# src-d/kmcuda

Hardware: AMD Instinct MI355X
Metric: point-assignments/sec per Lloyd iter (8Mx256@1024) (higher is better)
Workload: dtype f32

## Files before the change

kmcuda_amd/csrc/update.hip:

```cpp
#include <stdio.h>
#include <stdlib.h>
#include <string.h>

#include <algorithm>

#include <rocprim/device/device_radix_sort.hpp>

#include "exact.hpp"
#include "kernels.hpp"

namespace kmx {

static unsigned bits_for(uint64_t maxval) {
  unsigned b = 1;
  while (b < 32 && (1ull << b) <= maxval) b++;
  return b;
}

size_t sort_temp_bytes(size_t n, uint32_t max_key) {
  size_t bytes = 0;
  (void)rocprim::radix_sort_pairs(nullptr, bytes, (const uint32_t *)nullptr, (uint32_t *)nullptr,
                                  (const uint32_t *)nullptr, (uint32_t *)nullptr, n, 0u, bits_for(max_key),
                                  (hipStream_t)0);
  return bytes;
}

__global__ void offsets_kernel(const uint32_t *__restrict__ keys_sorted, uint32_t n, uint32_t nkeys,
                               uint32_t *__restrict__ offsets) {
  const uint32_t k = blockIdx.x * blockDim.x + threadIdx.x;
  if (k > nkeys) return;
  uint32_t lo = 0, hi = n;
  while (lo < hi) {
    const uint32_t mid = lo + (hi - lo) / 2;
    if (keys_sorted[mid] < k) lo = mid + 1; else hi = mid;
  }
  offsets[k] = lo;
}

__global__ void cluster_keys_kernel(const uint32_t *__restrict__ assignments, uint32_t N, uint32_t K,
                                    uint32_t *__restrict__ keys, uint32_t *__restrict__ vals) {
  const uint32_t s = blockIdx.x * blockDim.x + threadIdx.x;
  if (s >= N) return;
  const uint32_t a = assignments[s];
  keys[s] = a < K ? a : K;
  vals[s] = s;
}

hipError_t launch_inverse_assignments(const uint32_t *assignments, uint32_t N, uint32_t K, uint32_t *keys_tmp,
                                      uint32_t *vals_tmp, uint32_t *keys_sorted, uint32_t *inv,
                                      uint32_t *offsets, void *temp, size_t temp_bytes, hipStream_t st) {
  hipLaunchKernelGGL(cluster_keys_kernel, dim3((N + 255) / 256), dim3(256), 0, st, assignments, N, K, keys_tmp,
                     vals_tmp);
  hipError_t e = rocprim::radix_sort_pairs(temp, temp_bytes, (const uint32_t *)keys_tmp, keys_sorted,
                                           (const uint32_t *)vals_tmp, inv, (size_t)N, 0u, bits_for(K), st);
  if (e != hipSuccess) return e;
  hipLaunchKernelGGL(offsets_kernel, dim3((K + 1 + 255) / 256), dim3(256), 0, st, keys_sorted, N, K, offsets);
  return hipGetLastError();
}

__global__ void knn_query_keys_kernel(const float *__restrict__ lb, size_t stride, const uint32_t *__restrict__ offsets,
                                      uint32_t K, uint32_t p_base, uint32_t p_end, uint32_t *__restrict__ keys,
                                      uint32_t *__restrict__ vals, int mode, const float *__restrict__ mydist,
                                      const float *__restrict__ R) {
  const uint32_t i = blockIdx.x * blockDim.x + threadIdx.x;
  if (i >= p_end - p_base) return;
  const uint32_t p = p_base + i;
  uint32_t lo = 0, hi = K;
  while (hi - lo > 1) {
    const uint32_t mid = (lo + hi) / 2;
    if (offsets[mid] <= p) lo = mid; else hi = mid;
  }
  const uint32_t cls = lo;
  vals[i] = p;
  if (mode == 2) {
    const float md = mydist[p];
    const uint32_t q = (md == md && md > 0.f) ? ((__float_as_uint(md) >> 16) & 0x7FFFu) : 0u;
    keys[i] = (cls << 15) | q;
    return;
  }
  float best = INFINITY;
  uint32_t arg = 0;
  for (uint32_t c = 0; c < K; c++) {
    const float v = lb[(size_t)c * stride + i];
    if (c != cls && v < best) { best = v; arg = c; }
  }
  if (mode == 3) {
    const float r = R[cls], md = mydist[p];
    uint32_t q = 0;
    if (r > 0.f && md == md) q = (uint32_t)fminf(63.f, fmaxf(0.f, md / r * 63.f));
    keys[i] = ((cls * K + arg) << 6) | q;
    return;
  }
  keys[i] = cls * K + arg;
}

bool launch_knn_query_order(const float *lb, size_t stride, const uint32_t *offsets, uint32_t K, uint32_t p_base,
                            uint32_t p_end, uint32_t *keys_tmp, uint32_t *vals_tmp, uint32_t *keys_sorted,
                            uint32_t *qperm, void *temp, size_t temp_bytes, hipStream_t st, int mode,
                            const float *mydist, const float *R) {
  if (p_end <= p_base || K > 65535u) return false;
  const uint64_t key_max = mode == 2 ? ((uint64_t)K << 15) : (mode == 3 ? ((uint64_t)K * K) << 6 : (uint64_t)K * K);
  if (key_max > 0xFFFFFFFFull) return false;
  const uint32_t n = p_end - p_base;
  size_t need = 0;
  if (rocprim::radix_sort_pairs(nullptr, need, (const uint32_t *)nullptr, (uint32_t *)nullptr, (const uint32_t *)nullptr,
                                (uint32_t *)nullptr, (size_t)n, 0u, bits_for(key_max), st) != hipSuccess ||
      need > temp_bytes)
    return false;
  hipLaunchKernelGGL(knn_query_keys_kernel, dim3((n + 255) / 256), dim3(256), 0, st, lb, stride, offsets, K, p_base,
                     p_end, keys_tmp, vals_tmp, mode, mydist, R);
  size_t bytes = temp_bytes;
  return rocprim::radix_sort_pairs(temp, bytes, (const uint32_t *)keys_tmp, keys_sorted, (const uint32_t *)vals_tmp,
                                   qperm, (size_t)n, 0u, bits_for(key_max), st) == hipSuccess &&
         hipGetLastError() == hipSuccess;
}

__global__ void knn_probe_keys_kernel(const uint32_t *__restrict__ probes, uint32_t pw, const uint32_t *__restrict__ qinv,
                                      const uint32_t *__restrict__ offsets, uint32_t K, uint32_t p_base, uint32_t p_end,
                                      uint32_t *__restrict__ keys, uint32_t *__restrict__ vals) {
  const uint32_t i = blockIdx.x * blockDim.x + threadIdx.x;
  if (i >= p_end - p_base) return;
  const uint32_t p = p_base + i;
  uint32_t lo = 0, hi = K;
  while (hi - lo > 1) {
    const uint32_t mid = (lo + hi) / 2;
    if (offsets[mid] <= p) lo = mid; else hi = mid;
  }
  const uint32_t second = probes[(size_t)qinv[p] * pw + 1];
  vals[i] = p;
  keys[i] = lo * (K + 1) + (second < K ? second : K);
}

bool launch_knn_probe_order(const uint32_t *probes, uint32_t pw, const uint32_t *qinv, const uint32_t *offsets,
                            uint32_t K, uint32_t p_base, uint32_t p_end, uint32_t *keys_tmp, uint32_t *vals_tmp,
                            uint32_t *keys_sorted, uint32_t *qperm, void *temp, size_t temp_bytes, hipStream_t st) {
  if (p_end <= p_base || pw < 2 || K > 65535u) return false;
  const uint64_t key_max = (uint64_t)K * (K + 1);
  if (key_max > 0xFFFFFFFFull) return false;
  const uint32_t n = p_end - p_base;
  size_t need = 0;
  if (rocprim::radix_sort_pairs(nullptr, need, (const uint32_t *)nullptr, (uint32_t *)nullptr, (const uint32_t *)nullptr,
                                (uint32_t *)nullptr, (size_t)n, 0u, bits_for(key_max), st) != hipSuccess ||
      need > temp_bytes)
    return false;
  hipLaunchKernelGGL(knn_probe_keys_kernel, dim3((n + 255) / 256), dim3(256), 0, st, probes, pw, qinv, offsets, K, p_base,
                     p_end, keys_tmp, vals_tmp);
  size_t bytes = temp_bytes;
  return rocprim::radix_sort_pairs(temp, bytes, (const uint32_t *)keys_tmp, keys_sorted, (const uint32_t *)vals_tmp,
                                   qperm, (size_t)n, 0u, bits_for(key_max), st) == hipSuccess &&
         hipGetLastError() == hipSuccess;
}

__global__ void move_events_kernel(const uint32_t *__restrict__ prev, const uint32_t *__restrict__ cur, uint32_t N,
                                   uint32_t K, uint32_t *__restrict__ keys, uint32_t *__restrict__ vals) {
  const uint32_t s = blockIdx.x * blockDim.x + threadIdx.x;
  if (s >= N) return;
  const uint32_t p = prev[s], a = cur[s];
  const bool moved = p != a;
  const uint32_t sentinel = 2u * K;
  keys[2 * (size_t)s] = (moved && a < K) ? 2u * a : sentinel;
  keys[2 * (size_t)s + 1] = (moved && p < K) ? 2u * p + 1u : sentinel;
  vals[2 * (size_t)s] = s;
  vals[2 * (size_t)s + 1] = s;
}

constexpr uint32_t kMoveRows = 1024;

__device__ __forceinline__ void move_flags(const uint32_t *__restrict__ prev, const uint32_t *__restrict__ cur,
                                           uint32_t s, uint32_t N, uint32_t K, uint32_t &p, uint32_t &a, bool &ein,
                                           bool &eout) {
  p = a = 0;
  ein = eout = false;
  if (s < N) {
    p = prev[s];
    a = cur[s];
    const bool moved = p != a;
    ein = moved && a < K;
    eout = moved && p < K;
  }
}

__global__ __launch_bounds__(256) void move_count_kernel(const uint32_t *__restrict__ prev,
                                                         const uint32_t *__restrict__ cur, uint32_t N, uint32_t K,
                                                         uint32_t *__restrict__ blockcnt) {
  uint32_t cnt = 0;
#pragma unroll
  for (uint32_t i = 0; i < kMoveRows / 256; i++) {
    uint32_t p, a;
    bool ein, eout;
    move_flags(prev, cur, blockIdx.x * kMoveRows + i * 256 + threadIdx.x, N, K, p, a, ein, eout);
    cnt += (uint32_t)ein + (uint32_t)eout;
  }
#pragma unroll
  for (int o = 32; o > 0; o >>= 1) cnt += __shfl_xor(cnt, o);
  __shared__ uint32_t w[4];
  if ((threadIdx.x & 63) == 0) w[threadIdx.x >> 6] = cnt;
  __syncthreads();
  if (threadIdx.x == 0) blockcnt[blockIdx.x] = w[0] + w[1] + w[2] + w[3];
}

__global__ __launch_bounds__(1024) void move_scan_kernel(uint32_t *__restrict__ blockcnt, uint32_t nb,
                                                         uint32_t *__restrict__ total) {
  __shared__ uint32_t wsum[16];
  __shared__ uint32_t carry_s;
  const uint32_t lane = threadIdx.x & 63, wave = threadIdx.x >> 6;
  if (threadIdx.x == 0) carry_s = 0;
  __syncthreads();
  for (uint32_t base = 0; base < nb; base += 1024) {
    const uint32_t i = base + threadIdx.x;
    const uint32_t v = i < nb ? blockcnt[i] : 0u;
    uint32_t inc = v;
#pragma unroll
    for (int o = 1; o < 64; o <<= 1) {
      const uint32_t t = __shfl_up(inc, o);
      if ((int)lane >= o) inc += t;
    }
    if (lane == 63) wsum[wave] = inc;
    __syncthreads();
    uint32_t wbase = 0, all = 0;
#pragma unroll
    for (uint32_t k = 0; k < 16; k++) {
      const uint32_t t = wsum[k];
      if (k < wave) wbase += t;
      all += t;
    }
    const uint32_t carry = carry_s;
    if (i < nb) blockcnt[i] = carry + wbase + inc - v;
    __syncthreads();
    if (threadIdx.x == 0) carry_s = carry + all;
    __syncthreads();
  }
  if (threadIdx.x == 0) total[0] = carry_s;
}

__global__ __launch_bounds__(256) void move_write_kernel(const uint32_t *__restrict__ prev,
                                                         const uint32_t *__restrict__ cur, uint32_t N, uint32_t K,
                                                         const uint32_t *__restrict__ blockoff,
                                                         uint32_t *__restrict__ keys, uint32_t *__restrict__ vals) {
  __shared__ uint32_t wcnt[4];
  const uint32_t lane = threadIdx.x & 63, wave = threadIdx.x >> 6;
  uint32_t off = blockoff[blockIdx.x];
#pragma unroll
  for (uint32_t i = 0; i < kMoveRows / 256; i++) {
    const uint32_t s = blockIdx.x * kMoveRows + i * 256 + threadIdx.x;
    uint32_t p, a;
    bool ein, eout;
    move_flags(prev, cur, s, N, K, p, a, ein, eout);
    const unsigned long long min = __ballot(ein), mout = __ballot(eout);
    const unsigned long long lower = (1ull << lane) - 1ull;
    const uint32_t rank = (uint32_t)__popcll(min & lower) + (uint32_t)__popcll(mout & lower);
    if (lane == 0) wcnt[wave] = (uint32_t)__popcll(min) + (uint32_t)__popcll(mout);
    __syncthreads();
    uint32_t wbase = 0, all = 0;
#pragma unroll
    for (uint32_t k = 0; k < 4; k++) {
      if (k < wave) wbase += wcnt[k];
      all += wcnt[k];
    }
    const size_t at = (size_t)off + wbase + rank;
    if (ein) { keys[at] = 2u * a; vals[at] = s; }
    if (eout) { keys[at + (ein ? 1 : 0)] = 2u * p + 1u; vals[at + (ein ? 1 : 0)] = s; }
    off += all;
    __syncthreads();
  }
}

constexpr uint32_t kSumThreads = 1024;
constexpr uint32_t kBucketCapMax = 4096;

uint32_t move_bucket_cap(uint32_t N, uint32_t K) {
  uint32_t cap = 32;
  while (cap < kBucketCapMax && (uint64_t)cap * 2 * K <= (uint64_t)N) cap <<= 1;
  return cap;
}

struct SumArgs {
  const float *samples;
  uint32_t N, D, K;
  const uint32_t *prev, *cur;
  uint32_t *cursors;
  uint32_t stride;
  const uint32_t *bucket_rows;
  uint32_t cap;
  uint32_t *overflow;
  const uint32_t *rows_sorted, *offsets2;
  double *delta;
  int32_t *dcount;
  double *tail;
  const uint32_t *counters;
  uint32_t *res;
  uint32_t *host;
};

template <bool WEIGHTED>
__device__ __forceinline__ double list_sum(const float *__restrict__ samples, const float *__restrict__ weights,
                                           uint32_t D, const uint32_t *rows, uint32_t r0, uint32_t r1, uint32_t f) {
  double a[8] = {0, 0, 0, 0, 0, 0, 0, 0};
  uint32_t r = r0;
  for (; r + 8 <= r1; r += 8) {
    float x[8], w[8];
#pragma unroll
    for (int j = 0; j < 8; j++) {
      const uint32_t row = rows[r + j];
      x[j] = samples[(size_t)row * D + f];
      if constexpr (WEIGHTED) w[j] = weights[row];
    }
#pragma unroll
    for (int j = 0; j < 8; j++) {
      if constexpr (WEIGHTED) a[j] += (double)w[j] * (double)x[j];
      else a[j] += (double)x[j];
    }
  }
  for (uint32_t j = 0; r < r1; r++, j++) {
    const uint32_t row = rows[r];
    if constexpr (WEIGHTED) a[j] += (double)weights[row] * (double)samples[(size_t)row * D + f];
    else a[j] += (double)samples[(size_t)row * D + f];
  }
  return ((a[0] + a[1]) + (a[2] + a[3])) + ((a[4] + a[5]) + (a[6] + a[7]));
}

template <bool WEIGHTED>
__device__ __forceinline__ void list_sum4(const float *__restrict__ samples, const float *__restrict__ weights,
                                          uint32_t D, const uint32_t *rows, uint32_t r0, uint32_t r1, uint32_t f,
                                          double (&out)[4]) {
  double a[4][4];
#pragma unroll
  for (int j = 0; j < 4; j++)
#pragma unroll
    for (int e = 0; e < 4; e++) a[j][e] = 0.0;
  uint32_t r = r0;
  for (; r + 4 <= r1; r += 4) {
    float4 x[4];
    double w[4] = {1.0, 1.0, 1.0, 1.0};
#pragma unroll
    for (int j = 0; j < 4; j++) {
      const uint32_t row = rows[r + j];
      x[j] = *reinterpret_cast<const float4 *>(samples + (size_t)row * D + f);
      if constexpr (WEIGHTED) w[j] = (double)weights[row];
    }
#pragma unroll
    for (int j = 0; j < 4; j++) {
      if constexpr (WEIGHTED) {
        a[j][0] += w[j] * (double)x[j].x; a[j][1] += w[j] * (double)x[j].y;
        a[j][2] += w[j] * (double)x[j].z; a[j][3] += w[j] * (double)x[j].w;
      } else {
        a[j][0] += (double)x[j].x; a[j][1] += (double)x[j].y; a[j][2] += (double)x[j].z; a[j][3] += (double)x[j].w;
      }
    }
  }
  for (uint32_t j = 0; r < r1; r++, j++) {
    const uint32_t row = rows[r];
    float4 x = *reinterpret_cast<const float4 *>(samples + (size_t)row * D + f);
    double x0 = (double)x.x, x1 = (double)x.y, x2 = (double)x.z, x3 = (double)x.w;
    if constexpr (WEIGHTED) {
      const double w = (double)weights[row];
      x0 *= w; x1 *= w; x2 *= w; x3 *= w;
    }
    if (j == 0) { a[0][0] += x0; a[0][1] += x1; a[0][2] += x2; a[0][3] += x3; }
    else if (j == 1) { a[1][0] += x0; a[1][1] += x1; a[1][2] += x2; a[1][3] += x3; }
    else { a[2][0] += x0; a[2][1] += x1; a[2][2] += x2; a[2][3] += x3; }
  }
#pragma unroll
  for (int e = 0; e < 4; e++) out[e] = (a[0][e] + a[1][e]) + (a[2][e] + a[3][e]);
}

struct SumWeightArgs {
  const float *weights;
  double *dweight;
  double *win;
};

template <bool DIRECT, bool VEC4, bool WEIGHTED>
__device__ __forceinline__ void cluster_sums_body(const SumArgs &a, const SumWeightArgs &wa) {
  extern __shared__ __attribute__((aligned(16))) unsigned char sums_lds[];
  double *part = reinterpret_cast<double *>(sums_lds);
  uint32_t (*srt)[kBucketCapMax] = reinterpret_cast<uint32_t (*)[kBucketCapMax]>(sums_lds + kSumThreads * 4 * sizeof(double));
  uint32_t *part_u = reinterpret_cast<uint32_t *>(part);
  __shared__ uint32_t wcnt[16];
  __shared__ uint32_t sh_base;
  const uint32_t c = blockIdx.x, tid = threadIdx.x, lane = tid & 63, wave = tid >> 6;
  const uint32_t D = a.D;
  const uint32_t *rows[2];
  uint32_t n[2];
  if (DIRECT) {
    n[0] = a.cursors[(size_t)(2 * c) * a.stride];
    n[1] = a.cursors[(size_t)(2 * c + 1) * a.stride];
    __syncthreads();
    if (tid < 2) a.cursors[(size_t)(2 * c + tid) * a.stride] = 0u;
#pragma unroll
    for (int sg = 0; sg < 2; sg++) {
      const uint32_t cnt = n[sg], key = 2 * c + sg;
      if (cnt <= kSumThreads && cnt <= a.cap) {
        uint32_t *v = srt[sg];
        const uint32_t mine = tid < cnt ? a.bucket_rows[(size_t)key * a.cap + tid] : 0xFFFFFFFFu;
        if (tid < cnt) part_u[tid] = mine;
        __syncthreads();
        if (tid < cnt) {
          uint32_t rank = 0;
          for (uint32_t j = 0; j < cnt; j++) rank += part_u[j] < mine ? 1u : 0u;
          v[rank] = mine;
        }
        __syncthreads();
        rows[sg] = v;
      } else if (cnt <= a.cap) {
        uint32_t m = 2;
        while (m < cnt) m <<= 1;
        uint32_t *v = srt[sg];
        for (uint32_t i = tid; i < m; i += kSumThreads) v[i] = i < cnt ? a.bucket_rows[(size_t)key * a.cap + i] : 0xFFFFFFFFu;
        __syncthreads();
        if (cnt > 1) {
          for (uint32_t k = 2; k <= m; k <<= 1) {
            for (uint32_t j = k >> 1; j > 0; j >>= 1) {
              for (uint32_t i = tid; i < m; i += kSumThreads) {
                const uint32_t l = i ^ j;
                if (l > i) {
                  const uint32_t x = v[i], y = v[l];
                  const bool up = (i & k) == 0;
                  if ((x > y) == up) { v[i] = y; v[l] = x; }
                }
              }
              __syncthreads();
            }
          }
        }
        rows[sg] = v;
      } else {
        if (tid == 0) sh_base = atomicAdd(&a.res[3], cnt);
        __syncthreads();
        uint32_t *dst = a.overflow + sh_base;
        uint32_t done = 0;
        for (uint32_t base = 0; base < a.N; base += 4 * kSumThreads) {
          uint32_t hit[4], cntme = 0;
#pragma unroll
          for (uint32_t q = 0; q < 4; q++) {
            const uint32_t s = base + tid * 4 + q;
            uint32_t p, cu;
            bool ein, eout;
            move_flags(a.prev, a.cur, s, a.N, a.K, p, cu, ein, eout);
            const bool mine = sg == 0 ? (ein && cu == c) : (eout && p == c);
            hit[q] = mine ? s : 0xFFFFFFFFu;
            cntme += mine ? 1u : 0u;
          }
          uint32_t inc = cntme;
#pragma unroll
          for (int o = 1; o < 64; o <<= 1) {
            const uint32_t t = __shfl_up(inc, o);
            if ((int)lane >= o) inc += t;
          }
          if (lane == 63) wcnt[wave] = inc;
          __syncthreads();
          uint32_t wbase = 0, all = 0;
#pragma unroll
          for (uint32_t k = 0; k < 16; k++) {
            const uint32_t t = wcnt[k];
            if (k < wave) wbase += t;
            all += t;
          }
          uint32_t at = done + wbase + inc - cntme;
#pragma unroll
          for (uint32_t q = 0; q < 4; q++)
            if (hit[q] != 0xFFFFFFFFu) dst[at++] = hit[q];
          done += all;
          __syncthreads();
        }
        __threadfence_block();
        rows[sg] = dst;
      }
    }
    __syncthreads();
  } else {
    const uint32_t o0 = a.offsets2[2 * c], o1 = a.offsets2[2 * c + 1], o2 = a.offsets2[2 * c + 2];
    n[0] = o1 - o0; n[1] = o2 - o1;
    rows[0] = a.rows_sorted + o0;
    rows[1] = a.rows_sorted + o1;
  }

  double wsum[2] = {0.0, 0.0};
  if constexpr (WEIGHTED) {
#pragma unroll
    for (int sg = 0; sg < 2; sg++) {
      double t = 0.0;
      for (uint32_t r = tid; r < n[sg]; r += kSumThreads) t += (double)wa.weights[rows[sg][r]];
      part[sg * kSumThreads + tid] = t;
    }
    __syncthreads();
    if (wave == 0) {
#pragma unroll
      for (int sg = 0; sg < 2; sg++) {
        double t = part[sg * kSumThreads + lane];
        for (uint32_t k = 1; k < kSumThreads / 64; k++) t += part[sg * kSumThreads + k * 64 + lane];
#pragma unroll
        for (int o = 32; o > 0; o >>= 1) t += __shfl_xor(t, o);
        wsum[sg] = t;
      }
    }
    __syncthreads();
  }

  if (VEC4 && max(n[0], n[1]) >= 128u) {
    uint32_t fl = 16;
    while (fl < 256u && fl * 4u < D) fl <<= 1;
    const uint32_t groups = kSumThreads / fl, g = tid / fl, lf = tid % fl;
    for (uint32_t f0 = 0; f0 < D; f0 += 4u * fl) {
      const uint32_t f = f0 + 4u * lf;
      const bool fv = f < D;
      double tot[2][4];
#pragma unroll
      for (int sg = 0; sg < 2; sg++) {
        const uint32_t cnt = n[sg], chunk = (cnt + groups - 1) / groups;
        const uint32_t r0 = min(cnt, g * chunk), r1 = min(cnt, r0 + chunk);
        double mine[4] = {0.0, 0.0, 0.0, 0.0};
        if (fv && r1 > r0) list_sum4<WEIGHTED>(a.samples, wa.weights, D, rows[sg], r0, r1, f, mine);
#pragma unroll
        for (int e = 0; e < 4; e++) part[(size_t)tid * 4 + e] = mine[e];
        __syncthreads();
        if (g == 0) {
#pragma unroll
          for (int e = 0; e < 4; e++) {
            double t = part[(size_t)lf * 4 + e];
            for (uint32_t gg = 1; gg < groups; gg++) t += part[(size_t)(gg * fl + lf) * 4 + e];
            tot[sg][e] = t;
          }
        }
        __syncthreads();
      }
      if (g == 0 && fv) {
#pragma unroll
        for (int e = 0; e < 4; e++) a.delta[(size_t)c * D + f + e] = tot[0][e] - tot[1][e];
      }
    }
  } else {
  const uint32_t fl = D > 128 ? 256u : (D > 64 ? 128u : 64u), groups = kSumThreads / fl;
  const uint32_t g = tid / fl, lf = tid % fl;
  for (uint32_t f0 = 0; f0 < D; f0 += fl) {
    const uint32_t f = f0 + lf;
    const bool fv = f < D;
    double tot[2] = {0, 0};
#pragma unroll
    for (int sg = 0; sg < 2; sg++) {
      const uint32_t cnt = n[sg], chunk = (cnt + groups - 1) / groups;
      const uint32_t r0 = min(cnt, g * chunk), r1 = min(cnt, r0 + chunk);
      part[tid] = (fv && r1 > r0) ? list_sum<WEIGHTED>(a.samples, wa.weights, D, rows[sg], r0, r1, f) : 0.0;
      __syncthreads();
      if (g == 0) {
        double t = part[lf];
        for (uint32_t gg = 1; gg < groups; gg++) t += part[gg * fl + lf];
        tot[sg] = t;
      }
      __syncthreads();
    }
    if (g == 0 && fv) a.delta[(size_t)c * D + f] = tot[0] - tot[1];
  }
  }
  if (tid == 0) {
    const int32_t dc = (int32_t)n[0] - (int32_t)n[1];
    if (a.dcount) a.dcount[c] = dc;
    if (a.tail) a.tail[c] = (double)dc;
    if constexpr (WEIGHTED) {
      wa.dweight[c] = wsum[0] - wsum[1];
      wa.win[c] = wsum[0];
    }
    atomicAdd(&a.res[0], n[0] + n[1]);
    atomicMax(&a.res[1], max(n[0], n[1]));
    __threadfence();
    const uint32_t ticket = atomicAdd(&a.res[2], 1u);
    if (ticket == gridDim.x - 1) {
      if (a.counters[kStopFlag] == 0u) {
        volatile uint32_t *h = a.host;
        h[0] = atomicAdd(&a.res[0], 0u);
        h[1] = atomicAdd(&a.res[1], 0u);
        h[2] = a.counters[4];
        h[4] = a.counters[kDuoCount];
      }
      a.res[0] = 0u; a.res[1] = 0u; a.res[2] = 0u; a.res[3] = 0u;
    }
  }
  if (a.tail && c == 0 && tid < 4) a.tail[a.K + tid] = (double)a.counters[tid];
}

template <bool DIRECT, bool VEC4>
__global__ __launch_bounds__(kSumThreads) void cluster_sums_kernel(SumArgs a) {
  cluster_sums_body<DIRECT, VEC4, false>(a, SumWeightArgs{nullptr, nullptr, nullptr});
}
template <bool DIRECT, bool VEC4>
__global__ __launch_bounds__(kSumThreads) void cluster_sums_w_kernel(SumArgs a, SumWeightArgs wa) {
  cluster_sums_body<DIRECT, VEC4, true>(a, wa);
}

__global__ __launch_bounds__(256) void weight_changed_kernel(const double *__restrict__ win, uint32_t K,
                                                             double *__restrict__ out) {
  __shared__ double red[256];
  double t = 0.0;
  for (uint32_t c = threadIdx.x; c < K; c += 256) t += win[c];
  red[threadIdx.x] = t;
  __syncthreads();
  for (uint32_t s = 128; s > 0; s >>= 1) {
    if (threadIdx.x < s) red[threadIdx.x] += red[threadIdx.x + s];
    __syncthreads();
  }
  if (threadIdx.x == 0) out[0] = red[0];
}

constexpr uint32_t kWeightBlocks = 1024;
__global__ __launch_bounds__(256) void weights_check_kernel(const float *__restrict__ w, uint32_t N, uint32_t chunk,
                                                            double *__restrict__ part) {
  __shared__ double red[256], bad[256];
  const uint32_t lo = blockIdx.x * chunk, hi = min(N, lo + chunk);
  double t = 0.0, b = 0.0;
  for (uint32_t s = lo + threadIdx.x; s < hi; s += 256) {
    const float v = w[s];
    if (v > 0.f && v < INFINITY) t += (double)v; else b += 1.0;
  }
  red[threadIdx.x] = t; bad[threadIdx.x] = b;
  __syncthreads();
  for (uint32_t s = 128; s > 0; s >>= 1) {
    if (threadIdx.x < s) { red[threadIdx.x] += red[threadIdx.x + s]; bad[threadIdx.x] += bad[threadIdx.x + s]; }
    __syncthreads();
  }
  if (threadIdx.x == 0) { part[2 * blockIdx.x] = red[0]; part[2 * blockIdx.x + 1] = bad[0]; }
}
__global__ __launch_bounds__(256) void weights_total_kernel(const double *__restrict__ part, uint32_t nb,
                                                            double *__restrict__ out) {
  __shared__ double red[256], bad[256];
  double t = 0.0, b = 0.0;
  for (uint32_t i = threadIdx.x; i < nb; i += 256) { t += part[2 * i]; b += part[2 * i + 1]; }
  red[threadIdx.x] = t; bad[threadIdx.x] = b;
  __syncthreads();
  for (uint32_t s = 128; s > 0; s >>= 1) {
    if (threadIdx.x < s) { red[threadIdx.x] += red[threadIdx.x + s]; bad[threadIdx.x] += bad[threadIdx.x + s]; }
    __syncthreads();
  }
  if (threadIdx.x == 0) { out[0] = red[0]; out[1] = bad[0]; }
}
size_t weights_check_doubles() { return 2 * (size_t)kWeightBlocks + 2; }
hipError_t launch_weights_check(const float *weights, uint32_t N, double *work, hipStream_t st) {
  const uint32_t chunk = ((N + kWeightBlocks - 1) / kWeightBlocks + 255u) / 256u * 256u;
  const uint32_t nb = chunk ? (N + chunk - 1) / chunk : 0;
  if (nb) hipLaunchKernelGGL(weights_check_kernel, dim3(nb), dim3(256), 0, st, weights, N, chunk, work + 2);
  hipLaunchKernelGGL(weights_total_kernel, dim3(1), dim3(256), 0, st, work + 2, nb, work);
  return hipGetLastError();
}

uint32_t move_bucket_stride(uint32_t K) {
  uint32_t s = 32;
  while (s > 1 && 2ull * K * s > 262144ull) s >>= 1;
  return s;
}
size_t move_bucket_words(uint32_t K) { return 2 * (size_t)K * move_bucket_stride(K) + 4; }

__global__ __launch_bounds__(256) void move_scatter_kernel(const uint32_t *__restrict__ prev,
                                                           const uint32_t *__restrict__ cur, uint32_t N, uint32_t K,
                                                           uint32_t *__restrict__ cursors, uint32_t stride,
                                                           uint32_t *__restrict__ bucket_rows, uint32_t cap) {
  const uint32_t s = blockIdx.x * 256u + threadIdx.x;
  uint32_t p, a;
  bool ein, eout;
  move_flags(prev, cur, s, N, K, p, a, ein, eout);
  if (ein) {
    const uint32_t at = atomicAdd(&cursors[(size_t)(2u * a) * stride], 1u);
    if (at < cap) bucket_rows[(size_t)(2u * a) * cap + at] = s;
  }
  if (eout) {
    const uint32_t at = atomicAdd(&cursors[(size_t)(2u * p + 1u) * stride], 1u);
    if (at < cap) bucket_rows[(size_t)(2u * p + 1u) * cap + at] = s;
  }
}

hipError_t launch_move_deltas(const float *samples, uint32_t N, uint32_t D, uint32_t K, const uint32_t *prev,
                              const uint32_t *cur, uint32_t *keys_tmp, uint32_t *vals_tmp, uint32_t *keys_sorted,
                              uint32_t *rows_sorted, uint32_t *offsets2, void *temp, size_t temp_bytes,
                              uint32_t *bucket_rows, uint32_t cap, double *delta, int32_t *dcount, double *tail,
                              const uint32_t *counters, uint32_t *blockoff, uint32_t *bucket_work, MoveState *ms,
                              hipStream_t st, const MoveWeights *mw) {
  const uint32_t stride = move_bucket_stride(K);
  SumArgs a;
  a.samples = samples; a.N = N; a.D = D; a.K = K; a.prev = prev; a.cur = cur;
  a.cursors = bucket_work; a.stride = stride; a.bucket_rows = bucket_rows; a.cap = cap;
  a.overflow = rows_sorted; a.rows_sorted = rows_sorted; a.offsets2 = offsets2;
  a.delta = delta; a.dcount = dcount; a.tail = tail; a.counters = counters;
  a.res = bucket_work + 2 * (size_t)K * stride; a.host = ms->host_dev;
  hipError_t e = hipSuccess;
  const bool vec4 = (D & 3u) == 0 && (((uintptr_t)samples) & 15u) == 0;
  const size_t sums_lds = kSumThreads * 4 * sizeof(double) + 2 * kBucketCapMax * sizeof(uint32_t);
  auto launch_sums = [&](bool direct) {
    if (mw) {
      const SumWeightArgs wa{mw->weights, mw->dweight, mw->win};
      const void *fn = direct ? (vec4 ? (const void *)cluster_sums_w_kernel<true, true> : (const void *)cluster_sums_w_kernel<true, false>)
                              : (vec4 ? (const void *)cluster_sums_w_kernel<false, true> : (const void *)cluster_sums_w_kernel<false, false>);
      if (hipFuncSetAttribute(fn, hipFuncAttributeMaxDynamicSharedMemorySize, (int)sums_lds) != hipSuccess) return;
      if (direct) {
        if (vec4) hipLaunchKernelGGL((cluster_sums_w_kernel<true, true>), dim3(K), dim3(kSumThreads), sums_lds, st, a, wa);
        else hipLaunchKernelGGL((cluster_sums_w_kernel<true, false>), dim3(K), dim3(kSumThreads), sums_lds, st, a, wa);
      } else {
        if (vec4) hipLaunchKernelGGL((cluster_sums_w_kernel<false, true>), dim3(K), dim3(kSumThreads), sums_lds, st, a, wa);
        else hipLaunchKernelGGL((cluster_sums_w_kernel<false, false>), dim3(K), dim3(kSumThreads), sums_lds, st, a, wa);
      }
      hipLaunchKernelGGL(weight_changed_kernel, dim3(1), dim3(256), 0, st, mw->win, K, mw->dweight + K);
      return;
    }
    const void *fn = direct ? (vec4 ? (const void *)cluster_sums_kernel<true, true> : (const void *)cluster_sums_kernel<true, false>)
                            : (vec4 ? (const void *)cluster_sums_kernel<false, true> : (const void *)cluster_sums_kernel<false, false>);
    if (hipFuncSetAttribute(fn, hipFuncAttributeMaxDynamicSharedMemorySize, (int)sums_lds) != hipSuccess) return;
    if (direct) {
      if (vec4) hipLaunchKernelGGL((cluster_sums_kernel<true, true>), dim3(K), dim3(kSumThreads), sums_lds, st, a);
      else hipLaunchKernelGGL((cluster_sums_kernel<true, false>), dim3(K), dim3(kSumThreads), sums_lds, st, a);
    } else {
      if (vec4) hipLaunchKernelGGL((cluster_sums_kernel<false, true>), dim3(K), dim3(kSumThreads), sums_lds, st, a);
      else hipLaunchKernelGGL((cluster_sums_kernel<false, false>), dim3(K), dim3(kSumThreads), sums_lds, st, a);
    }
  };
  const bool force_radix = ms->force == 1, force_sync = ms->force == 2, force_direct = ms->force == 3;
  const uint32_t est_max = std::max((uint32_t)ms->host[1] , ms->last_events / K);
  const bool radix = N != 0 && !force_direct &&
                     (force_radix || ms->last_events > N / 2 || est_max > cap - cap / 4);
  if (N == 0) {
    e = hipMemsetAsync(offsets2, 0, (2 * (size_t)K + 1) * sizeof(uint32_t), st);
    if (e != hipSuccess) return e;
    launch_sums(false);
  } else if (radix) {
    ms->n_radix++;
    const uint32_t nb = (N + kMoveRows - 1) / kMoveRows;
    hipLaunchKernelGGL(move_count_kernel, dim3(nb), dim3(256), 0, st, prev, cur, N, K, blockoff);
    hipLaunchKernelGGL(move_scan_kernel, dim3(1), dim3(1024), 0, st, blockoff, nb, blockoff + nb + 1);
    hipLaunchKernelGGL(move_write_kernel, dim3(nb), dim3(256), 0, st, prev, cur, N, K, blockoff, keys_tmp, vals_tmp);
    e = hipGetLastError();
    if (e != hipSuccess) return e;
    e = hipMemcpyAsync(ms->host + 3, blockoff + nb + 1, sizeof(uint32_t), hipMemcpyDeviceToHost, st);
    if (e == hipSuccess) e = hipStreamSynchronize(st);
    if (e != hipSuccess) return e;
    const uint32_t m = ms->host[3];
    if (m) {
      e = rocprim::radix_sort_pairs(temp, temp_bytes, (const uint32_t *)keys_tmp, keys_sorted,
                                    (const uint32_t *)vals_tmp, rows_sorted, (size_t)m, 0u, bits_for(2ull * K), st);
      if (e != hipSuccess) return e;
    }
    hipLaunchKernelGGL(offsets_kernel, dim3((2 * K + 1 + 255) / 256), dim3(256), 0, st, keys_sorted, m, 2 * K, offsets2);
    ms->last_events = m;
    ms->host[0] = m;
    launch_sums(false);
  } else {
    ms->n_direct++;
    hipLaunchKernelGGL(move_scatter_kernel, dim3((N + 255) / 256), dim3(256), 0, st, prev, cur, N, K, bucket_work,
                       stride, bucket_rows, cap);
    launch_sums(true);
    e = hipGetLastError();
    if (e != hipSuccess) return e;
    if (force_sync) {
      e = hipStreamSynchronize(st);
      if (e != hipSuccess) return e;
    }
    ms->last_events = ms->host[0];
  }
  return hipGetLastError();
}

template <int METRIC, bool WEIGHTED>
__device__ __forceinline__ void apply_delta_body(const double *__restrict__ delta, const int32_t *__restrict__ dcount,
                                                 const double *__restrict__ dcount_d, uint32_t D,
                                                 float *__restrict__ centroids, uint32_t *__restrict__ ccounts,
                                                 const StopCtl &ctl, const double *__restrict__ wtail,
                                                 double *__restrict__ cweights) {
  const uint32_t c = blockIdx.x;
  if (ctl.counters) {
    bool stop = ctl.counters[kStopFlag] != 0u;
    if constexpr (WEIGHTED) {
      if (ctl.threshold >= 0.f && dcount_d) stop = stop || (float)wtail[gridDim.x] <= ctl.threshold;
    } else {
      if (ctl.threshold >= 0.f && dcount_d) stop = stop || (float)(uint32_t)dcount_d[gridDim.x] <= ctl.threshold;
    }
    if (c == 0 && threadIdx.x == 0) {
      if (stop) ctl.counters[kStopFlag] = 1u;
      else if (ctl.threshold >= 0.f) ctl.counters[0] = 0u;
      if (ctl.host_tail) {
        volatile uint32_t *ht = ctl.host_tail;
        for (uint32_t i = 0; i < 4; i++) ht[i] = dcount_d ? (uint32_t)dcount_d[gridDim.x + i] : 0u;
        ht[4] = stop ? 1u : 0u;
        __threadfence_system();
        ht[5] = ctl.seq;
      }
    }
    if (stop) return;
  }
  const double *d = delta + (size_t)c * D;
  float *cen = centroids + (size_t)c * D;
  const uint32_t cnt_old = ccounts[c];
  const uint32_t cnt_new = cnt_old + (uint32_t)(dcount_d ? (int32_t)dcount_d[c] : dcount[c]);
  double w, cn;
  if constexpr (WEIGHTED) {
    w = cnt_old ? cweights[c] : 0.0;
    cn = w + wtail[c];
  } else {
    w = (double)cnt_old;
    cn = (double)cnt_new;
  }
  if (cnt_new == 0) {
    for (uint32_t f = threadIdx.x; f < D; f += blockDim.x) cen[f] = __builtin_nanf("");
  } else if (METRIC == 0) {
    for (uint32_t f = threadIdx.x; f < D; f += blockDim.x) cen[f] = (float)(((double)cen[f] * w + d[f]) / cn);
  } else {
    __shared__ double red[256];
    double a = 0;
    for (uint32_t f = threadIdx.x; f < D; f += blockDim.x) {
      const double v = (double)cen[f] * w + d[f];
      a += v * v;
    }
    red[threadIdx.x] = a;
    __syncthreads();
    for (uint32_t s = blockDim.x / 2; s > 0; s >>= 1) {
      if (threadIdx.x < s) red[threadIdx.x] += red[threadIdx.x + s];
      __syncthreads();
    }
    const double nrm = sqrt(red[0]);
    for (uint32_t f = threadIdx.x; f < D; f += blockDim.x) cen[f] = (float)(((double)cen[f] * w + d[f]) / nrm);
  }
  __syncthreads();
  if (threadIdx.x == 0) {
    ccounts[c] = cnt_new;
    if constexpr (WEIGHTED) cweights[c] = cnt_new ? cn : 0.0;
  }
}

template <int METRIC>
__global__ void apply_delta_kernel(const double *__restrict__ delta, const int32_t *__restrict__ dcount,
                                   const double *__restrict__ dcount_d, uint32_t D, float *__restrict__ centroids,
                                   uint32_t *__restrict__ ccounts, StopCtl ctl) {
  apply_delta_body<METRIC, false>(delta, dcount, dcount_d, D, centroids, ccounts, ctl, nullptr, nullptr);
}
template <int METRIC>
__global__ void apply_delta_w_kernel(const double *__restrict__ delta, const int32_t *__restrict__ dcount,
                                     const double *__restrict__ dcount_d, uint32_t D, float *__restrict__ centroids,
                                     uint32_t *__restrict__ ccounts, StopCtl ctl, const double *__restrict__ wtail,
                                     double *__restrict__ cweights) {
  apply_delta_body<METRIC, true>(delta, dcount, dcount_d, D, centroids, ccounts, ctl, wtail, cweights);
}

hipError_t launch_apply_delta(int metric, const double *delta, const int32_t *dcount, const double *dcount_d,
                              uint32_t K, uint32_t D, float *centroids, uint32_t *ccounts, const StopCtl &stop,
                              hipStream_t st, const double *wtail, double *cweights) {
  const uint32_t bs = D >= 256 ? 256 : (D > 64 ? 128 : 64);
  if (wtail) {
    if (metric == 0)
      hipLaunchKernelGGL((apply_delta_w_kernel<0>), dim3(K), dim3(bs), 0, st, delta, dcount, dcount_d, D, centroids,
                         ccounts, stop, wtail, cweights);
    else
      hipLaunchKernelGGL((apply_delta_w_kernel<1>), dim3(K), dim3(bs), 0, st, delta, dcount, dcount_d, D, centroids,
                         ccounts, stop, wtail, cweights);
    return hipGetLastError();
  }
  if (metric == 0)
    hipLaunchKernelGGL((apply_delta_kernel<0>), dim3(K), dim3(bs), 0, st, delta, dcount, dcount_d, D, centroids, ccounts,
                       stop);
  else
    hipLaunchKernelGGL((apply_delta_kernel<1>), dim3(K), dim3(bs), 0, st, delta, dcount, dcount_d, D, centroids, ccounts,
                       stop);
  return hipGetLastError();
}

__global__ __launch_bounds__(256) void sum_buffers_kernel(double *const *__restrict__ bufs, uint32_t nbuf, size_t len) {
  for (size_t i = (size_t)blockIdx.x * 256 + threadIdx.x; i < len; i += (size_t)gridDim.x * 256) {
    double a = bufs[0][i];
    for (uint32_t b = 1; b < nbuf; b++) a += bufs[b][i];
    for (uint32_t b = 0; b < nbuf; b++) bufs[b][i] = a;
  }
}
hipError_t launch_sum_buffers(double *const *bufs_dev, uint32_t nbuf, size_t len, hipStream_t st) {
  const uint32_t grid = (uint32_t)std::min<size_t>((len + 255) / 256, 2048);
  hipLaunchKernelGGL(sum_buffers_kernel, dim3(grid ? grid : 1), dim3(256), 0, st, bufs_dev, nbuf, len);
  return hipGetLastError();
}

template <int METRIC, bool USE_LDS>
__global__ __launch_bounds__(64) void adjust_exact_kernel(const float *__restrict__ samples, uint32_t D, uint32_t K,
                                                          const uint32_t *__restrict__ rows,
                                                          const uint32_t *__restrict__ offsets,
                                                          float *__restrict__ centroids,
                                                          uint32_t *__restrict__ ccounts, float *__restrict__ work_g) {
  extern __shared__ float work_l[];
  float *work = USE_LDS ? work_l : work_g + (size_t)blockIdx.x * D * 64;
  const uint32_t lane = threadIdx.x;
  const uint32_t c = blockIdx.x * 64 + lane;
  const bool live = c < K;
  uint32_t my_count = live ? ccounts[c] : 0;
  float *cen = centroids + (size_t)(live ? c : 0) * D;
  {
    const float fmy = (float)my_count;
    for (uint32_t f = 0; f < D; f++) work[f * 64 + lane] = live ? cen[f] * fmy : 0.f;
  }
  uint32_t ia = live ? offsets[2 * c] : 0, ea = live ? offsets[2 * c + 1] : 0;
  uint32_t ib = ea, eb = live ? offsets[2 * c + 2] : 0;
  float corr = 0.f;
  while (ia < ea || ib < eb) {
    const uint32_t ra = ia < ea ? rows[ia] : 0xFFFFFFFFu;
    const uint32_t rb = ib < eb ? rows[ib] : 0xFFFFFFFFu;
    const bool in = ra < rb;
    const uint32_t row = in ? ra : rb;
    const float fsign = in ? 1.f : -1.f;
    if (in) { ia++; my_count++; } else { ib++; my_count--; }
    const float *x = samples + (size_t)row * D;
    uint32_t f = 0;
    if ((D & 3u) == 0) {
      for (; f < D; f += 4) {
        const float4 xv = *reinterpret_cast<const float4 *>(x + f);
        float c0 = work[(f + 0) * 64 + lane], c1 = work[(f + 1) * 64 + lane];
        float c2 = work[(f + 2) * 64 + lane], c3 = work[(f + 3) * 64 + lane];
        float y, t;
        y = fma_rd(xv.x, fsign, corr); t = c0 + y; corr = y - (t - c0); c0 = t;
        y = fma_rd(xv.y, fsign, corr); t = c1 + y; corr = y - (t - c1); c1 = t;
        y = fma_rd(xv.z, fsign, corr); t = c2 + y; corr = y - (t - c2); c2 = t;
        y = fma_rd(xv.w, fsign, corr); t = c3 + y; corr = y - (t - c3); c3 = t;
        work[(f + 0) * 64 + lane] = c0; work[(f + 1) * 64 + lane] = c1;
        work[(f + 2) * 64 + lane] = c2; work[(f + 3) * 64 + lane] = c3;
      }
    }
    for (; f < D; f++) {
      const float cv = work[f * 64 + lane];
      const float y = fma_rd(x[f], fsign, corr);
      const float t = cv + y;
      corr = y - (t - cv);
      work[f * 64 + lane] = t;
    }
  }
  if (!live) return;
  if (METRIC == 0) {
    const float rc = 1.0f / (float)my_count;
    for (uint32_t f = 0; f < D; f++) cen[f] = work[f * 64 + lane] * rc;
  } else {
    float norm = 0.f, ncorr = 0.f;
    for (uint32_t f = 0; f < D; f++) {
      const float v = work[f * 64 + lane];
      kahan_fold(fma_rd(v, v, ncorr), norm, ncorr);
    }
    norm = 1.0f / sqrtf(norm);
    for (uint32_t f = 0; f < D; f++) cen[f] = work[f * 64 + lane] * norm;
  }
  ccounts[c] = my_count;
}

hipError_t launch_adjust_exact(int metric, const float *samples, uint32_t N, uint32_t D, uint32_t K,
                               const uint32_t *prev, const uint32_t *cur, uint32_t *keys_tmp, uint32_t *vals_tmp,
                               uint32_t *keys_sorted, uint32_t *rows_sorted, uint32_t *offsets2, void *temp,
                               size_t temp_bytes, float *work, float *centroids, uint32_t *ccounts, hipStream_t st) {
  hipLaunchKernelGGL(move_events_kernel, dim3((N + 255) / 256), dim3(256), 0, st, prev, cur, N, K, keys_tmp, vals_tmp);
  hipError_t e = rocprim::radix_sort_pairs(temp, temp_bytes, (const uint32_t *)keys_tmp, keys_sorted,
                                           (const uint32_t *)vals_tmp, rows_sorted, 2 * (size_t)N, 0u,
                                           bits_for(2ull * K), st);
  if (e != hipSuccess) return e;
  hipLaunchKernelGGL(offsets_kernel, dim3((2 * K + 1 + 255) / 256), dim3(256), 0, st, keys_sorted, 2 * N, 2 * K,
                     offsets2);
  const uint32_t grid = (K + 63) / 64;
  const size_t lds = (size_t)D * 64 * sizeof(float);
  const bool use_lds = lds <= 128 * 1024;
#define KMX_ADJ(M, L)                                                                                        \
  hipLaunchKernelGGL((adjust_exact_kernel<M, L>), dim3(grid), dim3(64), (L) ? lds : 0, st, samples, D, K,    \
                     rows_sorted, offsets2, centroids, ccounts, work)
  if (use_lds) {
    e = hipFuncSetAttribute(metric == 0 ? (const void *)adjust_exact_kernel<0, true>
                                        : (const void *)adjust_exact_kernel<1, true>,
                            hipFuncAttributeMaxDynamicSharedMemorySize, (int)lds);
    if (e != hipSuccess) return e;
    if (metric == 0) KMX_ADJ(0, true); else KMX_ADJ(1, true);
  } else {
    if (metric == 0) KMX_ADJ(0, false); else KMX_ADJ(1, false);
  }
#undef KMX_ADJ
  return hipGetLastError();
}

hipError_t preload_update_code() {
  hipFuncAttributes at;
  return hipFuncGetAttributes(&at, reinterpret_cast<const void *>(&move_count_kernel));
}

}
```

Before: 2.202 billion.

## Restructure cluster sums kernel: merged barriers, wave-parallel ranking, deeper unrolled gathers

The list-sum helpers now unroll 16 (scalar) or 8 (float4) gathered rows per trip and handle the remainder with a masked tail, which puts more loads in flight. In the direct-bucket path, both subgroups' row IDs are loaded speculatively before the first barrier and ranked together, one wave per 64-row slice, using vectorised LDS reads. This replaces the per-subgroup serial ranking and its extra barriers. The delta reduction keeps both subgroups' partials in a doubled LDS buffer so it needs one barrier pair per feature tile instead of two, and the bookkeeping atomics are moved onto one thread inside the loop. In exchange the kernel uses more LDS and registers, which may lower occupancy.

```diff
diff --git a/kmcuda_amd/csrc/update.hip b/kmcuda_amd/csrc/update.hip
--- a/kmcuda_amd/csrc/update.hip
+++ b/kmcuda_amd/csrc/update.hip
@@ -295,26 +295,42 @@
 template <bool WEIGHTED>
 __device__ __forceinline__ double list_sum(const float *__restrict__ samples, const float *__restrict__ weights,
                                            uint32_t D, const uint32_t *rows, uint32_t r0, uint32_t r1, uint32_t f) {
+  constexpr int kTrip = 16;
   double a[8] = {0, 0, 0, 0, 0, 0, 0, 0};
+  const uint32_t full = (r1 - r0) / kTrip, rem = (r1 - r0) % kTrip;
   uint32_t r = r0;
-  for (; r + 8 <= r1; r += 8) {
-    float x[8], w[8];
-#pragma unroll
-    for (int j = 0; j < 8; j++) {
+  for (uint32_t t = 0; t < full; t++, r += kTrip) {
+    float x[kTrip], w[kTrip];
+#pragma unroll
+    for (int j = 0; j < kTrip; j++) {
       const uint32_t row = rows[r + j];
       x[j] = samples[(size_t)row * D + f];
       if constexpr (WEIGHTED) w[j] = weights[row];
     }
 #pragma unroll
-    for (int j = 0; j < 8; j++) {
-      if constexpr (WEIGHTED) a[j] += (double)w[j] * (double)x[j];
-      else a[j] += (double)x[j];
-    }
-  }
-  for (uint32_t j = 0; r < r1; r++, j++) {
-    const uint32_t row = rows[r];
-    if constexpr (WEIGHTED) a[j] += (double)weights[row] * (double)samples[(size_t)row * D + f];
-    else a[j] += (double)samples[(size_t)row * D + f];
+    for (int j = 0; j < kTrip; j++) {
+      if constexpr (WEIGHTED) a[j & 7] += (double)w[j] * (double)x[j];
+      else a[j & 7] += (double)x[j];
+    }
+  }
+  if (rem) {
+    float x[kTrip], w[kTrip];
+#pragma unroll
+    for (int j = 0; j < kTrip; j++) {
+      x[j] = 0.f; w[j] = 0.f;
+      if ((uint32_t)j < rem) {
+        const uint32_t row = rows[r + j];
+        x[j] = samples[(size_t)row * D + f];
+        if constexpr (WEIGHTED) w[j] = weights[row];
+      }
+    }
+#pragma unroll
+    for (int j = 0; j < kTrip; j++) {
+      if ((uint32_t)j < rem) {
+        if constexpr (WEIGHTED) a[j & 7] += (double)w[j] * (double)x[j];
+        else a[j & 7] += (double)x[j];
+      }
+    }
   }
   return ((a[0] + a[1]) + (a[2] + a[3])) + ((a[4] + a[5]) + (a[6] + a[7]));
 }
@@ -323,42 +339,60 @@
 __device__ __forceinline__ void list_sum4(const float *__restrict__ samples, const float *__restrict__ weights,
                                           uint32_t D, const uint32_t *rows, uint32_t r0, uint32_t r1, uint32_t f,
                                           double (&out)[4]) {
+  constexpr int kTrip = 8;
   double a[4][4];
 #pragma unroll
   for (int j = 0; j < 4; j++)
 #pragma unroll
     for (int e = 0; e < 4; e++) a[j][e] = 0.0;
+  const uint32_t full = (r1 - r0) / kTrip, rem = (r1 - r0) % kTrip;
   uint32_t r = r0;
-  for (; r + 4 <= r1; r += 4) {
-    float4 x[4];
-    double w[4] = {1.0, 1.0, 1.0, 1.0};
-#pragma unroll
-    for (int j = 0; j < 4; j++) {
+  for (uint32_t t = 0; t < full; t++, r += kTrip) {
+    float4 x[kTrip];
+    float w[kTrip];
+#pragma unroll
+    for (int j = 0; j < kTrip; j++) {
       const uint32_t row = rows[r + j];
       x[j] = *reinterpret_cast<const float4 *>(samples + (size_t)row * D + f);
-      if constexpr (WEIGHTED) w[j] = (double)weights[row];
-    }
-#pragma unroll
-    for (int j = 0; j < 4; j++) {
+      if constexpr (WEIGHTED) w[j] = weights[row];
+    }
+#pragma unroll
+    for (int j = 0; j < kTrip; j++) {
       if constexpr (WEIGHTED) {
-        a[j][0] += w[j] * (double)x[j].x; a[j][1] += w[j] * (double)x[j].y;
-        a[j][2] += w[j] * (double)x[j].z; a[j][3] += w[j] * (double)x[j].w;
+        const double wd = (double)w[j];
+        a[j & 3][0] += wd * (double)x[j].x; a[j & 3][1] += wd * (double)x[j].y;
+        a[j & 3][2] += wd * (double)x[j].z; a[j & 3][3] += wd * (double)x[j].w;
       } else {
-        a[j][0] += (double)x[j].x; a[j][1] += (double)x[j].y; a[j][2] += (double)x[j].z; a[j][3] += (double)x[j].w;
-      }
-    }
-  }
-  for (uint32_t j = 0; r < r1; r++, j++) {
-    const uint32_t row = rows[r];
-    float4 x = *reinterpret_cast<const float4 *>(samples + (size_t)row * D + f);
-    double x0 = (double)x.x, x1 = (double)x.y, x2 = (double)x.z, x3 = (double)x.w;
-    if constexpr (WEIGHTED) {
-      const double w = (double)weights[row];
-      x0 *= w; x1 *= w; x2 *= w; x3 *= w;
-    }
-    if (j == 0) { a[0][0] += x0; a[0][1] += x1; a[0][2] += x2; a[0][3] += x3; }
-    else if (j == 1) { a[1][0] += x0; a[1][1] += x1; a[1][2] += x2; a[1][3] += x3; }
-    else { a[2][0] += x0; a[2][1] += x1; a[2][2] += x2; a[2][3] += x3; }
+        a[j & 3][0] += (double)x[j].x; a[j & 3][1] += (double)x[j].y;
+        a[j & 3][2] += (double)x[j].z; a[j & 3][3] += (double)x[j].w;
+      }
+    }
+  }
+  if (rem) {
+    float4 x[kTrip];
+    float w[kTrip];
+#pragma unroll
+    for (int j = 0; j < kTrip; j++) {
+      x[j] = make_float4(0.f, 0.f, 0.f, 0.f); w[j] = 0.f;
+      if ((uint32_t)j < rem) {
+        const uint32_t row = rows[r + j];
+        x[j] = *reinterpret_cast<const float4 *>(samples + (size_t)row * D + f);
+        if constexpr (WEIGHTED) w[j] = weights[row];
+      }
+    }
+#pragma unroll
+    for (int j = 0; j < kTrip; j++) {
+      if ((uint32_t)j < rem) {
+        if constexpr (WEIGHTED) {
+          const double wd = (double)w[j];
+          a[j & 3][0] += wd * (double)x[j].x; a[j & 3][1] += wd * (double)x[j].y;
+          a[j & 3][2] += wd * (double)x[j].z; a[j & 3][3] += wd * (double)x[j].w;
+        } else {
+          a[j & 3][0] += (double)x[j].x; a[j & 3][1] += (double)x[j].y;
+          a[j & 3][2] += (double)x[j].z; a[j & 3][3] += (double)x[j].w;
+        }
+      }
+    }
   }
 #pragma unroll
   for (int e = 0; e < 4; e++) out[e] = (a[0][e] + a[1][e]) + (a[2][e] + a[3][e]);
@@ -374,7 +408,7 @@
 __device__ __forceinline__ void cluster_sums_body(const SumArgs &a, const SumWeightArgs &wa) {
   extern __shared__ __attribute__((aligned(16))) unsigned char sums_lds[];
   double *part = reinterpret_cast<double *>(sums_lds);
-  uint32_t (*srt)[kBucketCapMax] = reinterpret_cast<uint32_t (*)[kBucketCapMax]>(sums_lds + kSumThreads * 4 * sizeof(double));
+  uint32_t (*srt)[kBucketCapMax] = reinterpret_cast<uint32_t (*)[kBucketCapMax]>(sums_lds + 2 * kSumThreads * 4 * sizeof(double));
   uint32_t *part_u = reinterpret_cast<uint32_t *>(part);
   __shared__ uint32_t wcnt[16];
   __shared__ uint32_t sh_base;
@@ -383,25 +417,46 @@
   const uint32_t *rows[2];
   uint32_t n[2];
   if (DIRECT) {
-    n[0] = a.cursors[(size_t)(2 * c) * a.stride];
-    n[1] = a.cursors[(size_t)(2 * c + 1) * a.stride];
+    uint32_t spec[2];
+#pragma unroll
+    for (int sg = 0; sg < 2; sg++) {
+      n[sg] = __builtin_amdgcn_readfirstlane(a.cursors[(size_t)(2 * c + sg) * a.stride]);
+      spec[sg] = tid < a.cap ? a.bucket_rows[(size_t)(2 * c + sg) * a.cap + tid] : 0xFFFFFFFFu;
+    }
+    bool ranked[2];
+#pragma unroll
+    for (int sg = 0; sg < 2; sg++) {
+      ranked[sg] = n[sg] <= kSumThreads && n[sg] <= a.cap;
+      if (ranked[sg]) part_u[sg * kSumThreads + tid] = tid < n[sg] ? spec[sg] : 0xFFFFFFFFu;
+    }
     __syncthreads();
     if (tid < 2) a.cursors[(size_t)(2 * c + tid) * a.stride] = 0u;
+    for (uint32_t u = wave; u < 2 * (kSumThreads / 64); u += kSumThreads / 64) {
+      const uint32_t sg = u / (kSumThreads / 64);
+      const uint32_t vb = sg ? 2 * (kSumThreads / 64) - 1 - u : u;
+      const uint32_t cnt = n[sg];
+      if (!ranked[sg] || vb * 64 >= cnt) continue;
+      const uint32_t *vals = part_u + sg * kSumThreads;
+      const uint32_t mine = vals[vb * 64 + lane];
+      const uint4 *vals4 = reinterpret_cast<const uint4 *>(vals);
+      const uint32_t words = (cnt + 63) / 64 * 16;
+      uint32_t rank = 0;
+      for (uint32_t j = 0; j < words; j += 4) {
+        uint4 q[4];
+#pragma unroll
+        for (int i = 0; i < 4; i++) q[i] = vals4[j + i];
+#pragma unroll
+        for (int i = 0; i < 4; i++)
+          rank += (q[i].x < mine ? 1u : 0u) + (q[i].y < mine ? 1u : 0u) + (q[i].z < mine ? 1u : 0u) +
+                  (q[i].w < mine ? 1u : 0u);
+      }
+      if (vb * 64 + lane < cnt) srt[sg][rank] = mine;
+    }
 #pragma unroll
     for (int sg = 0; sg < 2; sg++) {
       const uint32_t cnt = n[sg], key = 2 * c + sg;
-      if (cnt <= kSumThreads && cnt <= a.cap) {
-        uint32_t *v = srt[sg];
-        const uint32_t mine = tid < cnt ? a.bucket_rows[(size_t)key * a.cap + tid] : 0xFFFFFFFFu;
-        if (tid < cnt) part_u[tid] = mine;
-        __syncthreads();
-        if (tid < cnt) {
-          uint32_t rank = 0;
-          for (uint32_t j = 0; j < cnt; j++) rank += part_u[j] < mine ? 1u : 0u;
-          v[rank] = mine;
-        }
-        __syncthreads();
-        rows[sg] = v;
+      if (ranked[sg]) {
+        rows[sg] = srt[sg];
       } else if (cnt <= a.cap) {
         uint32_t m = 2;
         while (m < cnt) m <<= 1;
@@ -469,14 +524,16 @@
     }
     __syncthreads();
   } else {
-    const uint32_t o0 = a.offsets2[2 * c], o1 = a.offsets2[2 * c + 1], o2 = a.offsets2[2 * c + 2];
+    const uint32_t o0 = __builtin_amdgcn_readfirstlane(a.offsets2[2 * c]);
+    const uint32_t o1 = __builtin_amdgcn_readfirstlane(a.offsets2[2 * c + 1]);
+    const uint32_t o2 = __builtin_amdgcn_readfirstlane(a.offsets2[2 * c + 2]);
     n[0] = o1 - o0; n[1] = o2 - o1;
     rows[0] = a.rows_sorted + o0;
     rows[1] = a.rows_sorted + o1;
   }
 
-  double wsum[2] = {0.0, 0.0};
   if constexpr (WEIGHTED) {
+    double wsum[2] = {0.0, 0.0};
 #pragma unroll
     for (int sg = 0; sg < 2; sg++) {
       double t = 0.0;
@@ -493,73 +550,18 @@
         for (int o = 32; o > 0; o >>= 1) t += __shfl_xor(t, o);
         wsum[sg] = t;
       }
-    }
-    __syncthreads();
-  }
-
-  if (VEC4 && max(n[0], n[1]) >= 128u) {
-    uint32_t fl = 16;
-    while (fl < 256u && fl * 4u < D) fl <<= 1;
-    const uint32_t groups = kSumThreads / fl, g = tid / fl, lf = tid % fl;
-    for (uint32_t f0 = 0; f0 < D; f0 += 4u * fl) {
-      const uint32_t f = f0 + 4u * lf;
-      const bool fv = f < D;
-      double tot[2][4];
-#pragma unroll
-      for (int sg = 0; sg < 2; sg++) {
-        const uint32_t cnt = n[sg], chunk = (cnt + groups - 1) / groups;
-        const uint32_t r0 = min(cnt, g * chunk), r1 = min(cnt, r0 + chunk);
-        double mine[4] = {0.0, 0.0, 0.0, 0.0};
-        if (fv && r1 > r0) list_sum4<WEIGHTED>(a.samples, wa.weights, D, rows[sg], r0, r1, f, mine);
-#pragma unroll
-        for (int e = 0; e < 4; e++) part[(size_t)tid * 4 + e] = mine[e];
-        __syncthreads();
-        if (g == 0) {
-#pragma unroll
-          for (int e = 0; e < 4; e++) {
-            double t = part[(size_t)lf * 4 + e];
-            for (uint32_t gg = 1; gg < groups; gg++) t += part[(size_t)(gg * fl + lf) * 4 + e];
-            tot[sg][e] = t;
-          }
-        }
-        __syncthreads();
-      }
-      if (g == 0 && fv) {
-#pragma unroll
-        for (int e = 0; e < 4; e++) a.delta[(size_t)c * D + f + e] = tot[0][e] - tot[1][e];
-      }
-    }
-  } else {
-  const uint32_t fl = D > 128 ? 256u : (D > 64 ? 128u : 64u), groups = kSumThreads / fl;
-  const uint32_t g = tid / fl, lf = tid % fl;
-  for (uint32_t f0 = 0; f0 < D; f0 += fl) {
-    const uint32_t f = f0 + lf;
-    const bool fv = f < D;
-    double tot[2] = {0, 0};
-#pragma unroll
-    for (int sg = 0; sg < 2; sg++) {
-      const uint32_t cnt = n[sg], chunk = (cnt + groups - 1) / groups;
-      const uint32_t r0 = min(cnt, g * chunk), r1 = min(cnt, r0 + chunk);
-      part[tid] = (fv && r1 > r0) ? list_sum<WEIGHTED>(a.samples, wa.weights, D, rows[sg], r0, r1, f) : 0.0;
-      __syncthreads();
-      if (g == 0) {
-        double t = part[lf];
-        for (uint32_t gg = 1; gg < groups; gg++) t += part[gg * fl + lf];
-        tot[sg] = t;
-      }
-      __syncthreads();
-    }
-    if (g == 0 && fv) a.delta[(size_t)c * D + f] = tot[0] - tot[1];
-  }
-  }
-  if (tid == 0) {
+      if (tid == 0) {
+        wa.dweight[c] = wsum[0] - wsum[1];
+        wa.win[c] = wsum[0];
+      }
+    }
+    __syncthreads();
+  }
+
+  auto bookkeeping = [&]() {
     const int32_t dc = (int32_t)n[0] - (int32_t)n[1];
     if (a.dcount) a.dcount[c] = dc;
     if (a.tail) a.tail[c] = (double)dc;
-    if constexpr (WEIGHTED) {
-      wa.dweight[c] = wsum[0] - wsum[1];
-      wa.win[c] = wsum[0];
-    }
     atomicAdd(&a.res[0], n[0] + n[1]);
     atomicMax(&a.res[1], max(n[0], n[1]));
     __threadfence();
@@ -574,6 +576,61 @@
       }
       a.res[0] = 0u; a.res[1] = 0u; a.res[2] = 0u; a.res[3] = 0u;
     }
+  };
+
+  if (VEC4 && max(n[0], n[1]) >= 128u) {
+    uint32_t fl = 16;
+    while (fl < 256u && fl * 4u < D) fl <<= 1;
+    const uint32_t groups = kSumThreads / fl, g = tid / fl, lf = tid % fl;
+    for (uint32_t f0 = 0; f0 < D; f0 += 4u * fl) {
+      const uint32_t f = f0 + 4u * lf;
+      const bool fv = f < D;
+#pragma unroll
+      for (int sg = 0; sg < 2; sg++) {
+        const uint32_t cnt = n[sg], chunk = (cnt + groups - 1) / groups;
+        const uint32_t r0 = min(cnt, g * chunk), r1 = min(cnt, r0 + chunk);
+        double mine[4] = {0.0, 0.0, 0.0, 0.0};
+        if (fv && r1 > r0) list_sum4<WEIGHTED>(a.samples, wa.weights, D, rows[sg], r0, r1, f, mine);
+#pragma unroll
+        for (int e = 0; e < 4; e++) part[(size_t)sg * 4 * kSumThreads + (size_t)tid * 4 + e] = mine[e];
+      }
+      __syncthreads();
+      if (f0 == 0 && tid == kSumThreads - 1) bookkeeping();
+      if (tid < 4u * fl) {
+        double t0 = part[tid], t1 = part[4 * kSumThreads + tid];
+        for (uint32_t gg = 1; gg < groups; gg++) {
+          t0 += part[(size_t)gg * 4 * fl + tid];
+          t1 += part[4 * kSumThreads + (size_t)gg * 4 * fl + tid];
+        }
+        if (f0 + tid < D) a.delta[(size_t)c * D + f0 + tid] = t0 - t1;
+      }
+      __syncthreads();
+    }
+  } else {
+  const uint32_t fl = D > 128 ? 256u : (D > 64 ? 128u : 64u), groups = kSumThreads / fl;
+  const uint32_t g = tid / fl, lf = tid % fl;
+  for (uint32_t f0 = 0; f0 < D; f0 += fl) {
+    const uint32_t f = f0 + lf;
+    const bool fv = f < D;
+#pragma unroll
+    for (int sg = 0; sg < 2; sg++) {
+      const uint32_t cnt = n[sg], chunk = (cnt + groups - 1) / groups;
+      const uint32_t r0 = min(cnt, g * chunk), r1 = min(cnt, r0 + chunk);
+      part[sg * kSumThreads + tid] =
+          (fv && r1 > r0) ? list_sum<WEIGHTED>(a.samples, wa.weights, D, rows[sg], r0, r1, f) : 0.0;
+    }
+    __syncthreads();
+    if (f0 == 0 && tid == kSumThreads - 1) bookkeeping();
+    if (g == 0) {
+      double t0 = part[lf], t1 = part[kSumThreads + lf];
+      for (uint32_t gg = 1; gg < groups; gg++) {
+        t0 += part[gg * fl + lf];
+        t1 += part[kSumThreads + gg * fl + lf];
+      }
+      if (fv) a.delta[(size_t)c * D + f] = t0 - t1;
+    }
+    __syncthreads();
+  }
   }
   if (a.tail && c == 0 && tid < 4) a.tail[a.K + tid] = (double)a.counters[tid];
 }
@@ -681,7 +738,7 @@
   a.res = bucket_work + 2 * (size_t)K * stride; a.host = ms->host_dev;
   hipError_t e = hipSuccess;
   const bool vec4 = (D & 3u) == 0 && (((uintptr_t)samples) & 15u) == 0;
-  const size_t sums_lds = kSumThreads * 4 * sizeof(double) + 2 * kBucketCapMax * sizeof(uint32_t);
+  const size_t sums_lds = 2 * kSumThreads * 4 * sizeof(double) + 2 * kBucketCapMax * sizeof(uint32_t);
   auto launch_sums = [&](bool direct) {
     if (mw) {
       const SumWeightArgs wa{mw->weights, mw->dweight, mw->win};
```

Result: no change. 2.198 billion (-0.2%).
